# QuentinHuan/ENSEM3A_OpenCLRaytracer

Hardware: NVIDIA B200
Metric: Mrays/s (higher is better)
Workload: dtype f32

## Files before the change

ensem3a_openclraytracer_b200/_capi.py:

```python
import ctypes
import os
import subprocess

import numpy as np

_PKG = os.path.dirname(os.path.abspath(__file__))
LIB_PATH = os.path.join(_PKG, "lib", "libb200rt.so")
CSRC = os.path.join(_PKG, "csrc")

RNG_REFERENCE, RNG_PHILOX = 0, 1
TRAVERSAL_FAST, TRAVERSAL_REFERENCE, TRAVERSAL_VERIFY = 0, 1, 2
OUT_FINAL, OUT_SUMS = 0, 1
SAMPLING_REFERENCE, SAMPLING_IMPORTANCE, SAMPLING_LIGHTS = 0, 1, 2


class B200RTError(RuntimeError):
    pass


class Opts(ctypes.Structure):
    _fields_ = [("rng_mode", ctypes.c_int32), ("traversal", ctypes.c_int32), ("stack_cap", ctypes.c_int32),
                ("output", ctypes.c_int32), ("sample_begin", ctypes.c_int32), ("sample_end", ctypes.c_int32),
                ("pixel_begin", ctypes.c_int32), ("pixel_end", ctypes.c_int32), ("seed", ctypes.c_uint64),
                ("collect_stats", ctypes.c_int32), ("time_kernels", ctypes.c_int32), ("tile_row_mod", ctypes.c_int32),
# ... 26 lines not shown

DENOISE_DEFAULTS = dict(passes=5, sigma_color=0.5, sigma_normal=0.2, sigma_position=0.0)


def _denoise_params(passes=DENOISE_DEFAULTS["passes"], sigma_color=DENOISE_DEFAULTS["sigma_color"],
                    sigma_normal=DENOISE_DEFAULTS["sigma_normal"], sigma_position=DENOISE_DEFAULTS["sigma_position"]):
    return Denoise(int(passes), float(sigma_color), float(sigma_normal), float(sigma_position))


SYMBOLS = [
    "b200rt_default_opts", "b200rt_create", "b200rt_destroy", "b200rt_last_error", "b200rt_set_scene",
    "b200rt_set_materials", "b200rt_set_ibl", "b200rt_render", "b200rt_render_adaptive", "b200rt_gbuffer", "b200rt_denoise", "b200rt_render_denoised", "b200rt_render_rgb8", "b200rt_render_device", "b200rt_finalize_device",
    "b200rt_reduce_finalize_device", "b200rt_sync", "b200rt_set_stream", "b200rt_invalidate", "b200rt_primary_hits", "b200rt_trace_rays",
    "b200rt_img_processing", "b200rt_get_stats", "b200rt_math_probe", "b200rt_philox_probe", "b200rt_alloc",
    "b200rt_free", "b200rt_ipc_export",
    "b200rt_ipc_open", "b200rt_ipc_close", "b200rt_build_bvh", "b200rt_repack_probe", "b200rt_version", "b200rt_device_count",
    "b200rt_multi_create", "b200rt_multi_destroy", "b200rt_multi_last_error", "b200rt_multi_device_count",
    "b200rt_multi_context", "b200rt_multi_set_scene", "b200rt_multi_set_ibl", "b200rt_multi_invalidate",
    "b200rt_multi_render", "b200rt_multi_render_denoised", "b200rt_multi_get_stats",
]

_lib = None


def build_library(verbose=False):
    cmd = ["make", "-C", CSRC] + ([] if verbose else ["-s"])
    subprocess.check_call(cmd)
    return LIB_PATH


def load_library():
# ... 32 lines not shown
    lib.b200rt_set_stream.argtypes = [vp, vp]
    lib.b200rt_invalidate.argtypes = [vp]
    lib.b200rt_primary_hits.argtypes = [vp, vp, i32, i32, ctypes.POINTER(Opts), vp, vp]
    lib.b200rt_trace_rays.argtypes = [vp, vp, i64, ctypes.POINTER(Opts), vp, vp]
    lib.b200rt_img_processing.argtypes = [vp, vp, vp, i64, i64]
    lib.b200rt_get_stats.argtypes = [vp, ctypes.POINTER(Stats)]
    lib.b200rt_math_probe.argtypes = [vp, i32, vp, vp, i64, vp]
    lib.b200rt_philox_probe.argtypes = [vp, ctypes.POINTER(u32 * 4), u32, u32, ctypes.POINTER(u32 * 4)]
    lib.b200rt_alloc.argtypes = [vp, i64, ctypes.POINTER(vp)]
    lib.b200rt_free.argtypes = [vp, vp]
    lib.b200rt_ipc_export.argtypes = [vp, vp, vp]
    lib.b200rt_ipc_open.argtypes = [vp, vp, ctypes.POINTER(vp)]
    lib.b200rt_ipc_close.argtypes = [vp, vp]
    lib.b200rt_build_bvh.argtypes = [vp, i64, vp, i64, vp, i64, ctypes.POINTER(ctypes.c_int32)]
    lib.b200rt_repack_probe.argtypes = [vp, i64, vp, i64, vp, i64, i64, vp, i64, vp, i64, vp, vp]
    lib.b200rt_multi_create.argtypes = [ctypes.POINTER(ctypes.c_int), i32, ctypes.POINTER(vp)]
    lib.b200rt_multi_destroy.restype = None
    lib.b200rt_multi_destroy.argtypes = [vp]
    lib.b200rt_multi_last_error.restype = ctypes.c_char_p
    lib.b200rt_multi_last_error.argtypes = [vp]
    lib.b200rt_multi_device_count.argtypes = [vp]
    lib.b200rt_multi_context.restype = vp
    lib.b200rt_multi_context.argtypes = [vp, i32]
    lib.b200rt_multi_set_scene.argtypes = [vp, vp, i64, vp, i64, vp, i64, vp, i64, vp, i64, vp, i64, vp, i64]
    lib.b200rt_multi_set_ibl.argtypes = [vp, vp, i32, i32]
    lib.b200rt_multi_invalidate.argtypes = [vp]
    lib.b200rt_multi_render.argtypes = [vp, vp, vp, i32, i32, i32, i32, ctypes.POINTER(Opts), vp]
    lib.b200rt_multi_get_stats.argtypes = [vp, ctypes.POINTER(Stats)]
    for name in SYMBOLS:
        fn = getattr(lib, name)
# ... 59 lines not shown
    if rc != 0:
        raise B200RTError(f"b200rt_repack_probe failed ({rc})")
    nodes = np.zeros((int(info[0]), 8), np.uint32)
    ranks = np.zeros(face.size // 10, np.int32)
    rc = lib.b200rt_repack_probe(_ptr(vp_), vp_.size, _ptr(vn_), vn_.size, _ptr(face), face.size, int(n_materials),
                                 _ptr(bvh_), bvh_.size, _ptr(nodes), nodes.size, _ptr(ranks), _ptr(info))
    if rc != 0:
        raise B200RTError(f"b200rt_repack_probe failed ({rc})")
    d = dict(n_inner=int(info[0]), node_f4=int(info[1]), depth=int(info[2]), ref_stack_need=int(info[3]),
             canonical=bool(info[4]), fast_ok=bool(info[5]), cmax=float(info[6]), cull_abs=float(info[7]),
             grid_base=info[8:11].copy(), grid_pitch=info[11:14].copy(), root_qmin=info[14:17].copy(),
             root_qmax=info[17:20].copy(), ranks=ranks, ms_tris=float(info[20]), ms_walk=float(info[21]), ms_nodes=float(info[22]), cull_depth=int(info[23]))
    return nodes, d


class _Handle:

    _prefix = "b200rt_"

    def __del__(self):
        try:
            self.close()
        except Exception:
            pass

    def _check(self, rc, what):
        if rc != 0:
            err = getattr(self._lib, self._prefix + "last_error")(self._h).decode()
            raise B200RTError(f"{what} failed ({rc}): {err}")

# ... 257 lines not shown
```

ensem3a_openclraytracer_b200/csrc/b200rt_api.cu:

```cuda
#include <cmath>
#include <cstdarg>
#include <cstdio>
#include <cstdlib>
#include <cstring>
#include <chrono>
#include <string>
#include <type_traits>
#include <vector>

#include "../../include/b200rt.h"
#include "rt_denoise.cuh"
#include "scene_repack.h"

using namespace b200rt;

namespace {

thread_local std::string g_create_error;

struct DevBuf {
  void *p = nullptr;
  size_t cap = 0;
  bool borrowed = false;
};
// ... 66 lines not shown
  vsnprintf(buf, sizeof buf, fmt, ap);
  va_end(ap);
  if (c) c->err = buf; else g_create_error = buf;
  return code;
}

#define CU(call)                                                                                   \
  do {                                                                                             \
    cudaError_t e_ = (call);                                                                       \
    if (e_ != cudaSuccess) return fail(c, B200RT_ERR_CUDA, "%s: %s", #call, cudaGetErrorString(e_)); \
  } while (0)

}

static_assert(kRefStack == kRefStackMax, "scene_repack.h and rt_trace.cuh disagree on the exact walk's stack");
size_t b200rt::lane_smem_bytes_host(int stack_depth) { return lane_smem_bytes(stack_depth); }

namespace {

int ensure(b200rt_ctx *c, DevBuf &b, size_t bytes) {
  if (bytes == 0) bytes = 16;
  if (b.borrowed) return fail(c, B200RT_ERR_INVALID, "internal: resize of a borrowed scene buffer");
  if (b.cap >= bytes) return 0;
  if (b.p) cudaFree(b.p);
  b.p = nullptr;
  b.cap = 0;
  CU(cudaMalloc(&b.p, bytes));
  b.cap = bytes;
  return 0;
}
// ... 50 lines not shown
  F->s0 = o.sample_begin;
  F->s1 = o.sample_end;
  if (F->s1 <= 0) { F->s0 = 0; F->s1 = spp; }
  F->pixel_begin = o.pixel_begin;
  F->pixel_end = o.pixel_end;
  if (F->pixel_end <= 0) { F->pixel_begin = 0; F->pixel_end = width * height; }
  F->tile_row_mod = o.tile_row_mod;
  F->tile_row_rem = o.tile_row_rem;
  F->out_mode = o.output;
  F->rng_mode = o.rng_mode;
  F->key0 = (uint32_t)(o.seed & 0xffffffffull);
  F->key1 = (uint32_t)(o.seed >> 32);
  F->sampling = o.sampling;
}

size_t scene_smem_bytes(const b200rt_ctx *c) { return (size_t)c->scene.n_inner * 48 + (size_t)c->scene.n_tris * 48; }

bool use_smem_scene(const b200rt_ctx *c) { return c->scene.node_f4 == 3; }

int stack_entries(const b200rt_ctx *c) { return c->scene.canonical ? c->scene.cull_depth + 2 : 2; }

size_t smem_bytes(const b200rt_ctx *c, bool smem_scene) {
  return lane_smem_bytes(stack_entries(c)) + (smem_scene ? scene_smem_bytes(c) : 0);
}

int effective_stack_cap(const b200rt_ctx *c, const b200rt_opts &o);

void fill_args(b200rt_ctx *c, const FrameParams &F, const b200rt_opts &o, float *d_out, KernelArgs *A) {
  A->F = F;
  const SceneDesc &D = c->scene;
  const DevBuf *B = c->d_scene;
  SceneView &S = A->S;
  S.nodes = static_cast<const uint4 *>(B[kNodes].p);
  S.node_f4 = D.node_f4;
  S.tris = static_cast<const float4 *>(B[kTris].p);
  S.ctris = static_cast<const float4 *>(B[kCtris].p);
  S.normals = static_cast<const float4 *>(B[kNormals].p);
  S.tboxes = static_cast<const float4 *>(B[kTboxes].p);
  S.frames = static_cast<const float4 *>(B[kFrames].p);
  S.mats = static_cast<const float *>(B[kMats].p);
  S.bvh9 = static_cast<const float *>(B[kBvh9].p);
  S.leafcnt = static_cast<const int *>(B[kLeafcnt].p);
  S.root_ref = D.root_ref;
  for (int i = 0; i < 3; ++i) {
    S.grid_base[i] = D.grid_base[i];
    S.grid_pitch[i] = D.grid_pitch[i];
    S.root_w[i] = D.root_w[i];
  }
  S.cull_abs = D.cull_abs;
  S.cmax = D.cmax;
  {
    const int E = std::ilogb((1001.0f + D.cull_abs) * 1.01f) + 1;
    S.st_bias = (uint32_t)(E - 32 + 127) << 23;
    unsigned long long m = 1;
    while (m < (unsigned long long)std::max(1, D.n_inner) * (unsigned long long)std::max(1, D.node_f4)) m <<= 1;
    S.st_rmask = (uint32_t)(m - 1ull);
  }
  S.stack_cap = effective_stack_cap(c, o);
  S.fast_ok = D.fast_ok;
  A->ibl = c->ibl_tex;
  A->prim_dirk = static_cast<float4 *>(c->d_prim_dirk.p);
  A->prim_tri = static_cast<int *>(c->d_prim_tri.p);
  A->out = d_out;
  A->pA = static_cast<float4 *>(c->d_pA.p);
  A->pB = static_cast<float4 *>(c->d_pB.p);
  A->pC = static_cast<float4 *>(c->d_pC.p);
  A->pHit = static_cast<int2 *>(c->d_pHit.p);
  A->light = static_cast<const int *>(B[kLight].p);
  A->n_light = c->n_light;
  A->pS = static_cast<float4 *>(c->d_pS.p);
  A->pL = static_cast<float4 *>(c->d_pL.p);
  A->pR = static_cast<float4 *>(c->d_pR.p);
  A->list[0] = static_cast<int *>(c->d_list0.p);
  A->list[1] = static_cast<int *>(c->d_list1.p);
  A->cnt = static_cast<unsigned int *>(c->d_cnt.p);
  A->slots = static_cast<int *>(c->d_slots.p);
  A->part_count = static_cast<unsigned int *>(c->d_part_count.p);
  A->wc = nullptr;
  A->counters = c->d_counters;
  A->n_nodes = D.n_inner;
  A->n_tris = D.n_tris;
  A->stack_depth = stack_entries(c);
  A->tiles_x = (F.width + 7) / 8;
  int tiles_y = (F.height + 3) / 4;
  A->n_work = A->tiles_x * tiles_y * 32;
  A->validate = 0;
  A->ad = AdaptArgs();
}

int effective_traversal(const b200rt_ctx *c, const b200rt_opts &o) {
  if (!c->scene.canonical) return B200RT_TRAVERSAL_REFERENCE;
  return o.traversal;
}

int effective_stack_cap(const b200rt_ctx *c, const b200rt_opts &o) {
// ... 619 lines not shown

bool scene_is_cached(const b200rt_ctx *c, uint64_t h) { return c->have_scene && c->have_scene_cached && h == c->scene_hash; }

int upload_scene(b200rt_ctx *c, const Repacked &R, const SceneArgs &a, uint64_t h) {
  c->have_scene = false;
  c->have_scene_cached = false;
  c->scene_hash = 0;
  const int n_tris = R.n_tris;
  DevBuf *B = c->d_scene;
  CU(cudaSetDevice(c->device));
  if (ensure(c, B[kTris], R.tris.size() * sizeof(float4))) return B200RT_ERR_CUDA;
  if (ensure(c, B[kCtris], R.ctris.size() * sizeof(float4))) return B200RT_ERR_CUDA;
  if (ensure(c, B[kNormals], R.normals.size() * sizeof(float4))) return B200RT_ERR_CUDA;
  if (ensure(c, B[kTboxes], R.tboxes.size() * sizeof(float4))) return B200RT_ERR_CUDA;
  if (ensure(c, B[kFrames], (size_t)n_tris * kFrameVec * sizeof(float4))) return B200RT_ERR_CUDA;
  if (ensure(c, B[kNodes], R.nodes.size() * sizeof(uint4))) return B200RT_ERR_CUDA;
  if (ensure(c, B[kBvh9], (size_t)a.n_bvh * 4)) return B200RT_ERR_CUDA;
  if (ensure(c, B[kLeafcnt], R.leaf_count.size() * sizeof(int32_t))) return B200RT_ERR_CUDA;
  CU(cudaMemcpyAsync(B[kLeafcnt].p, R.leaf_count.data(), R.leaf_count.size() * sizeof(int32_t), cudaMemcpyHostToDevice, c->stream));
  CU(cudaMemcpyAsync(B[kTris].p, R.tris.data(), R.tris.size() * sizeof(float4), cudaMemcpyHostToDevice, c->stream));
  CU(cudaMemcpyAsync(B[kCtris].p, R.ctris.data(), R.ctris.size() * sizeof(float4), cudaMemcpyHostToDevice, c->stream));
  CU(cudaMemcpyAsync(B[kNormals].p, R.normals.data(), R.normals.size() * sizeof(float4), cudaMemcpyHostToDevice, c->stream));
  CU(cudaMemcpyAsync(B[kTboxes].p, R.tboxes.data(), R.tboxes.size() * sizeof(float4), cudaMemcpyHostToDevice, c->stream));
  if (!R.nodes.empty())
    CU(cudaMemcpyAsync(B[kNodes].p, R.nodes.data(), R.nodes.size() * sizeof(uint4), cudaMemcpyHostToDevice, c->stream));
  CU(cudaMemcpyAsync(B[kBvh9].p, a.bvh, (size_t)a.n_bvh * 4, cudaMemcpyHostToDevice, c->stream));
  k_tri_frames<<<(n_tris + 127) / 128, 128, 0, c->stream>>>(static_cast<const float4 *>(B[kNormals].p), n_tris,
                                                           static_cast<float4 *>(B[kFrames].p));
  CU(cudaGetLastError());
  CU(cudaStreamSynchronize(c->stream));
  c->scene = R;
  c->tri_mat = R.tri_mat;
  c->mat_hash = 0;
  c->n_mats = 0;
  int rc = b200rt_set_materials(c, a.mat, a.n_mat);
  if (rc) return rc;
  c->have_scene = true;
  c->have_scene_cached = true;
  c->scene_hash = h;
  ++c->scene_epoch;
// ... 890 lines not shown
```

ensem3a_openclraytracer_b200/csrc/rt_kernels.cuh:

```cuda
#pragma once
#include "rt_shade.cuh"
#include "rt_trace.cuh"

namespace b200rt {

constexpr int kBlock = 128;
constexpr int kShadeBlock = 128;
constexpr unsigned kChunk = 32;
constexpr int kQuorum = 12, kRefillMin = 8, kTriQuorum = 2;
constexpr int kCompactEvery = 4;
constexpr int kHitNeedsExactWalk = -2;

struct DeviceCounters {
  unsigned long long rays, box_tests, tri_tests, mismatches, samples, revalidated, exact_walks, primary_rays;
};

struct AdaptArgs {
  float2 *welford;
  int *spp_out;
  float *err_out;
  int min_spp, check_every;
  float rel_error, floor;
};

// ... 563 lines not shown
  T.Q.A = mk3(1, 1, 1); T.Q.Bn = mk3(0, 0, 0); T.Q.Bf = mk3(0, 0, 0);
  for (int a = 0; a < 3; ++a) { T.Q.sn[a] = kSelMin; T.Q.sf[a] = kSelMax; }
  int pn = 0;
  int path = -1;
  unsigned int c_next = 0, c_end = 0;
  bool exhausted = false;

  unsigned int rays = 0;
  unsigned int mism = 0;
  TraceCounters tc;
  tc.box_tests = 0; tc.tri_tests = 0;

  int thresh = kQuorum;
  for (;;) {
    for (;;) {
      const bool can = trav_active(T) && pn <= kParkCap - 2;
      if (__popc(__ballot_sync(0xffffffffu, can)) < thresh) break;
      if (can) trav_step<SMEM, STATS>(S, T, pn, parks, kBlock, st, &tc);
    }
    for (unsigned int pm = __ballot_sync(0xffffffffu, pn > 0); pm != 0u;) {
      if (pn > 0) {
        --pn;
        if (STATS) tc.tri_tests++;
        test_parked<SMEM>(S, T, parks[pn * kBlock], T.o, T.d);
      }
      pm = __ballot_sync(0xffffffffu, pn > 0);
      if (__popc(pm) < kTriQuorum) break;
    }
    const bool finished = (path >= 0) && !trav_active(T) && pn == 0;
    if (finished) {
      A.pHit[path] = make_int2(T.best.tri, __float_as_int(T.best.k));
      path = -1;
    }
    const unsigned int idle = __ballot_sync(0xffffffffu, path < 0);
    if (exhausted) {
      if (idle == 0xffffffffu) break;
      continue;
    }
    const int n_idle = __popc(idle);
    if (n_idle == 0) continue;
    if (n_idle < kRefillMin &&
        __popc(__ballot_sync(0xffffffffu, trav_active(T) && pn <= kParkCap - 2)) >= kQuorum)
      continue;
    {
      int need = n_idle;
      int rank = __popc(idle & lt_mask);
      bool want = path < 0;
      while (need > 0) {
        if (c_next == c_end) {
          unsigned int b = 0;
          if (lane == 0) b = atomicAdd(wc, kChunk);
          b = __shfl_sync(0xffffffffu, b, 0);
          if (b >= n) { exhausted = true; thresh = 1; break; }
          c_next = b;
          c_end = min(b + kChunk, n);
        }
        const int take = min(need, (int)(c_end - c_next));
// ... 146 lines not shown
```

ensem3a_openclraytracer_b200/csrc/rt_trace.cuh:

```cuda
#pragma once
#include "rt_math.cuh"

namespace b200rt {

struct SceneView {
  const uint4 *nodes;
  int node_f4;
  const float4 *tris;
  const float4 *ctris;
  const float4 *normals;
  const float4 *tboxes;
  const float4 *frames;
  const float *mats;
  const float *bvh9;
  const int *leafcnt;
  int root_ref;
  float grid_base[3];
  float grid_pitch[3];
  uint32_t root_w[3];
  float cull_abs;
  uint32_t st_bias;
  uint32_t st_rmask;
  float cmax;
  int stack_cap;
// ... 40 lines not shown
  v3 A, e1, e2;
  int mat, rank, id;
};
template <bool SMEM = false>
RT_DEV Tri load_tri(const float4 *tris, int t) {
  const float4 *p = tris + 3 * (size_t)t;
  const float4 t0 = ld4<SMEM>(p), t1 = ld4<SMEM>(p + 1), t2 = ld4<SMEM>(p + 2);
  return {mk3(t0.x, t0.y, t0.z), mk3(t0.w, t1.x, t1.y), mk3(t1.z, t1.w, t2.x), __float_as_int(t2.y), __float_as_int(t2.z),
          __float_as_int(t2.w)};
}

RT_DEV int tri_material(const SceneView &S, int tri) { return __float_as_int(__ldg(S.tris + 3 * (size_t)tri + 2).y); }
RT_DEV int tri_rank(const SceneView &S, int tri) { return __float_as_int(__ldg(S.tris + 3 * (size_t)tri + 2).z); }

template <bool SMEM>
RT_DEV void ld_node(const uint4 *p, uint4 &a, uint4 &b) {
  if (SMEM) {
    a = p[0]; b = p[1];
  } else {
    asm("ld.global.nc.v8.u32 {%0,%1,%2,%3,%4,%5,%6,%7}, [%8];"
        : "=r"(a.x), "=r"(a.y), "=r"(a.z), "=r"(a.w), "=r"(b.x), "=r"(b.y), "=r"(b.z), "=r"(b.w)
        : "l"(p));
  }
}

constexpr uint32_t kSelMax = 0x7324u;
constexpr uint32_t kSelMin = 0x7104u;
RT_DEV float plane_fq(uint32_t w, uint32_t sel) {
  uint32_t r;
  asm("prmt.b32 %0, %1, %2, %3;" : "=r"(r) : "r"(w), "r"(0x3f000000u), "r"(sel));
  return __uint_as_float(r);
}

RT_DEV float div_exact(float x, float d) {
  if (x == 0.0f && d != 0.0f && d == d) return __uint_as_float((__float_as_uint(x) ^ __float_as_uint(d)) & 0x80000000u);
  return __fdiv_rn(x, d);
}

RT_DEV bool slab_exact(v3 o, v3 d, float mnx, float mny, float mnz, float mxx, float mxy, float mxz, float *tmin,
// ... 186 lines not shown
}

struct Trav {
  v3 o, d;
  RayFast Q;
  Hit best;
  int best_rank;
  float lim;
  int cur, sp;
};

RT_DEV bool trav_active(const Trav &T) { return T.cur >= 0; }

RT_DEV float cull_limit(const SceneView &S, const Trav &T) { return __fmaf_rn(T.best.k, 1.001f, S.cull_abs); }

constexpr int kParkCap = 6;

template <bool SMEM, bool STATS>
RT_DEV void trav_begin(const SceneView &S, Trav &T, v3 o, v3 d, int &pn, uint32_t *parks, TraceCounters *cnt) {
  T.o = o; T.d = d;
  T.Q = make_rayfast(S, o, d);
  T.best.tri = -1;
  T.best.k = 1000.0f;
  T.best_rank = 0x7fffffff;
  T.lim = cull_limit(S, T);
  T.sp = 0;
  float lo, hi;
  if (STATS) cnt->box_tests++;
  slab_cons(T.Q, S.root_w[0], S.root_w[1], S.root_w[2], &lo, &hi);
  const bool go = hi >= lo;
  T.cur = go ? 0 : -1;
  if (go && S.root_ref < 0) {
    parks[0] = (uint32_t)S.root_ref;
    pn = 1;
    T.cur = -1;
  }
}

template <bool SMEM, bool STATS>
RT_DEV void trav_step(const SceneView &S, Trav &T, int &pn, uint32_t *parks, int pstride, LaneStack st,
                      TraceCounters *cnt) {
  uint4 wa, wb;
  ld_node<SMEM>(S.nodes + T.cur, wa, wb);
  const int refL = (int)wb.z, refR = (int)wb.w;
  float loL, hiL, loR, hiR;
  if (STATS) cnt->box_tests += 2;
  slab_cons(T.Q, wa.x, wa.y, wa.z, &loL, &hiL);
  slab_cons(T.Q, wa.w, wb.x, wb.y, &loR, &hiR);
  const float lim = T.lim;
  const float behind = -S.cull_abs;
  const bool goL = hiL >= loL && !(loL > lim) && !(hiL < behind);
  const bool goR = hiR >= loR && !(loR > lim) && !(hiR < behind);
  const bool leafL = goL && refL < 0, leafR = goR && refR < 0;
  const bool inL = goL && refL >= 0, inR = goR && refR >= 0;
  const bool rNear = loR < loL;
  const int refNear = rNear ? refR : refL, refFar = rNear ? refL : refR;
  const bool both = leafL && leafR;
  if (both) { parks[pn * pstride] = (uint32_t)refFar; ++pn; }
  if (leafL || leafR) { parks[pn * pstride] = (uint32_t)(both ? refNear : (leafR ? refR : refL)); ++pn; }
  if (inL && inR) {
    st.base[T.sp * st.stride] = (stack_code(S, rNear ? loL : loR) & ~S.st_rmask) | (uint32_t)refFar;
    ++T.sp;
    T.cur = refNear;
  } else if (inL || inR) {
    T.cur = inL ? refL : refR;
  } else {
    T.cur = -1;
    const uint32_t keep = stack_code(S, lim) | S.st_rmask;
    while (T.sp > 0) {
      --T.sp;
      const uint32_t e = st.base[T.sp * st.stride];
      if (e <= keep) {
        T.cur = (int)(e & S.st_rmask);
        break;
      }
    }
  }
}

template <bool SMEM>
RT_DEV void test_parked(const SceneView &S, Trav &T, uint32_t ref, v3 o, v3 d) {
  test_triangle<SMEM>(S, ~(int)ref, o, d, T.best, T.best_rank);
  T.lim = cull_limit(S, T);
}

template <bool SMEM, bool STATS>
RT_DEV Hit closest_hit_fast(const SceneView &S, v3 o, v3 d, LaneStack st, uint32_t *parks, int pstride,
                            TraceCounters *cnt) {
  if (!ray_is_fast(S, o)) return closest_hit_nodrop(S, o, d);
  Trav T;
  int pn = 0;
  trav_begin<SMEM, STATS>(S, T, o, d, pn, parks, cnt);
  while (trav_active(T) || pn > 0) {
    if (pn > 0 && (!trav_active(T) || pn > kParkCap - 2)) {
      --pn;
      if (STATS) cnt->tri_tests++;
      test_parked<SMEM>(S, T, parks[pn * pstride], o, d);
    } else {
      trav_step<SMEM, STATS>(S, T, pn, parks, pstride, st, cnt);
    }
  }
  if (T.best.tri >= 0 && !validate_winner(S, o, d, T.best.tri, T.best_rank)) return closest_hit_nodrop(S, o, d);
  return T.best;
}

template <int TRAV, bool SMEM, bool STATS>
RT_DEV Hit closest_hit(const SceneView &S, v3 o, v3 d, LaneStack st, uint32_t *parks, int pstride, TraceCounters *cnt,
                       unsigned int *mismatch) {
  if (TRAV == 0) return closest_hit_fast<SMEM, STATS>(S, o, d, st, parks, pstride, cnt);
// ... 11 lines not shown
```

ensem3a_openclraytracer_b200/csrc/scene_repack.cpp:

```cpp
#include "scene_repack.h"

#include <omp.h>

#include <algorithm>
#include <chrono>
#include <cmath>
#include <cstdio>
#include <cstdlib>
#include <cstring>

#include "../../include/b200rt.h"

namespace b200rt {

namespace {

double now_ms() {
  return std::chrono::duration<double, std::milli>(std::chrono::steady_clock::now().time_since_epoch()).count();
}

std::string fmt(const char *f, long long a = 0, long long b = 0, long long c = 0) {
  char buf[256];
  snprintf(buf, sizeof buf, f, a, b, c);
  return buf;
// ... 40 lines not shown
    if (const char *q = getenv("B200RT_HOST_THREADS")) {
      want = atoi(q);
    } else if (omp_get_max_threads() == 1) {
      const char *omp = getenv("OMP_NUM_THREADS"), *lws = getenv("LOCAL_WORLD_SIZE");
      if (omp && lws && atoi(omp) == 1 && atoi(lws) >= 1) want = std::min(16, omp_get_num_procs() / atoi(lws));
    }
    if (want >= 1) {
      saved = omp_get_max_threads();
      omp_set_num_threads(want);
    }
  }
  ~HostThreads() {
    if (saved) omp_set_num_threads(saved);
  }
};

}

int repack_scene(const float *vp, int64_t n_vp, const float *vn, int64_t n_vn, const int32_t *face, int64_t n_face,
                 int64_t n_materials, const float *bvh, int64_t n_bvh, Repacked *out, std::string *err, bool own_tree) {
  HostThreads host_threads;
  Repacked &R = *out;
  const int n_nodes = (int)(n_bvh / 9), n_tris = (int)(n_face / 10);
  const int nvp = (int)(n_vp / 3), nvn = (int)(n_vn / 3), nm = (int)n_materials;
  R.n_nodes9 = n_nodes;
  R.n_tris = n_tris;
  double t0 = now_ms();

  R.tris.resize((size_t)n_tris * 3);
  R.normals.resize((size_t)n_tris);
// ... 222 lines not shown
    return B200RT_ERR_INVALID;
  }
  R.depth = depth;
  R.cull_depth = depth;
  R.cull_tree = 0;
  R.ref_stack_need = (int)max_stack;
  if (R.ref_stack_need > kRefStackMax) canonical = false;
  double t2 = now_ms();
  R.ms_walk = t2 - t1;

  std::vector<CullNode> cull;
  if (canonical && own_tree && T(0) == -1) {
    build_cull_tree(R.tboxes.data(), n_tris, &cull, &R.cull_depth);
    R.cull_tree = 1;
  }
  if (lane_smem_bytes_host(R.cull_depth + 2) > kLaneSmemMax) canonical = false;

  Axis grid[3];
  {
    double ext[3], ext_max = 0.0;
    for (int k = 0; k < 3; ++k) {
      ext[k] = std::max(0.0, (double)bvh[5 + k] - (double)bvh[2 + k]);
      ext_max = std::max(ext_max, ext[k]);
    }
    if (ext_max == 0.0) ext_max = std::max((double)cmax, 1e-30) * 0x1p-12;
    for (int k = 0; k < 3; ++k) {
      const double e = std::max(ext[k], ext_max / 256.0);
      double widen = 0x1p-20;
      for (int attempt = 0;; ++attempt) {
        float pitch = (float)(e * (65536.0 / 32767.0) * (1.0 + 8.0 * widen));
        if (!(pitch > 0.0f) || !std::isfinite(pitch)) pitch = 1.0f;
// ... 41 lines not shown
        todo.push_back(0);
        while (!todo.empty()) {
          const int cur = todo.back();
          todo.pop_back();
          const int ch[2] = {L(cur), Rc(cur)};
          for (int k = 0; k < 2; ++k)
            if (T(ch[k]) == -1) {
              inner_id[ch[k]] = (int)order.size();
              order.push_back(ch[k]);
            }
          for (int k = 1; k >= 0; --k)
            if (T(ch[k]) == -1) todo.push_back(ch[k]);
        }
      }
      }
      std::vector<int> leaf_pos;
      if (R.cull_tree) {
        leaf_pos.assign((size_t)n_tris, -1);
        int pos = 0;
        for (size_t q = 0; q < cull.size(); ++q)
          for (int k = 0; k < 2; ++k)
            if (cull[q].ref[k] < 0) leaf_pos[(size_t)~cull[q].ref[k]] = pos++;
      }
      const int n_inner = R.cull_tree ? (int)cull.size() : (int)order.size();
      R.n_inner = n_inner;
      const int nf4 = ((size_t)n_inner * 48 + (size_t)n_tris * 48 <= kSmemSceneMax) ? 3 : 2;
      R.node_f4 = nf4;
      R.nodes.resize((size_t)n_inner * nf4);
      int outside = 0;
#pragma omp parallel for schedule(static) reduction(| : outside)
      for (int q = 0; q < n_inner; ++q) {
        const float *bl, *br;
        int32_t refl, refr;
        if (R.cull_tree) {
          const CullNode &N = cull[q];
          bl = N.box[0]; br = N.box[1];
          refl = N.ref[0] < 0 ? ~leaf_pos[(size_t)~N.ref[0]] : N.ref[0] * nf4;
          refr = N.ref[1] < 0 ? ~leaf_pos[(size_t)~N.ref[1]] : N.ref[1] * nf4;
        } else {
          const int cur = order[q];
          const int l = L(cur), r = Rc(cur);
          bl = bvh + 9 * (size_t)l + 2; br = bvh + 9 * (size_t)r + 2;
          refl = T(l) != -1 ? ~T(l) : (int32_t)(inner_id[l] * nf4);
          refr = T(r) != -1 ? ~T(r) : (int32_t)(inner_id[r] * nf4);
        }
        uint32_t wl[3], wr[3];
        for (int k = 0; k < 3; ++k)
          if (!quantise(grid[k], bl[k], bl[3 + k], &wl[k]) || !quantise(grid[k], br[k], br[3 + k], &wr[k])) outside |= 1;
        Repacked::u4 a, b;
        a.x = wl[0]; a.y = wl[1]; a.z = wl[2]; a.w = wr[0];
        b.x = wr[1]; b.y = wr[2];
        b.z = (uint32_t)refl;
        b.w = (uint32_t)refr;
        R.nodes[(size_t)nf4 * q + 0] = a;
        R.nodes[(size_t)nf4 * q + 1] = b;
        if (nf4 == 3) R.nodes[(size_t)nf4 * q + 2] = Repacked::u4{0, 0, 0, 0};
      }
      if (R.cull_tree) {
        R.ctris.resize((size_t)n_tris * 3);
#pragma omp parallel for schedule(static)
        for (int t = 0; t < n_tris; ++t) {
          const size_t p = (size_t)leaf_pos[(size_t)t];
          R.ctris[3 * p] = R.tris[3 * (size_t)t];
          R.ctris[3 * p + 1] = R.tris[3 * (size_t)t + 1];
          Repacked::f4 t2 = R.tris[3 * (size_t)t + 2];
          t2.w = as_float((uint32_t)t);
          R.ctris[3 * p + 2] = t2;
        }
      }
      if (outside) {
        R.canonical = false;
        R.nodes.clear();
        R.n_inner = 0;
        R.node_f4 = 2;
      }
    }
  }
  if (R.ctris.size() != R.tris.size() || !R.cull_tree || !R.canonical) {
    R.ctris.resize(R.tris.size());
#pragma omp parallel for schedule(static)
    for (int t = 0; t < n_tris; ++t) {
      R.ctris[3 * (size_t)t] = R.tris[3 * (size_t)t];
      R.ctris[3 * (size_t)t + 1] = R.tris[3 * (size_t)t + 1];
      Repacked::f4 t2 = R.tris[3 * (size_t)t + 2];
      t2.w = as_float((uint32_t)t);
      R.ctris[3 * (size_t)t + 2] = t2;
    }
  }
  R.ms_nodes = now_ms() - t2;
  return 0;
}

}
// ... 12 lines not shown
  info[0] = (float)R.n_inner; info[1] = (float)R.node_f4; info[2] = (float)R.depth; info[3] = (float)R.ref_stack_need;
  info[4] = R.canonical ? 1.0f : 0.0f; info[5] = (float)R.fast_ok; info[6] = R.cmax; info[7] = R.cull_abs;
  for (int k = 0; k < 3; ++k) {
    info[8 + k] = R.grid_base[k]; info[11 + k] = R.grid_pitch[k];
    info[14 + k] = (float)(R.root_w[k] & 0xffffu); info[17 + k] = (float)(R.root_w[k] >> 16);
  }
  info[20] = (float)R.ms_tris; info[21] = (float)R.ms_walk; info[22] = (float)R.ms_nodes; info[23] = (float)R.cull_depth;
  if (rank_out)
    for (int t = 0; t < R.n_tris; ++t) memcpy(&rank_out[t], &R.tris[3 * (size_t)t + 2].z, 4);
  if (nodes_out) {
    if (n_nodes_out < (int64_t)R.n_inner * 8) return B200RT_ERR_INVALID;
    for (int q = 0; q < R.n_inner; ++q) {
      const b200rt::Repacked::u4 &a = R.nodes[(size_t)R.node_f4 * q], &b = R.nodes[(size_t)R.node_f4 * q + 1];
      uint32_t *o = nodes_out + 8 * (size_t)q;
      o[0] = a.x; o[1] = a.y; o[2] = a.z; o[3] = a.w; o[4] = b.x; o[5] = b.y; o[6] = b.z; o[7] = b.w;
      for (int k = 6; k < 8; ++k)
        if ((int32_t)o[k] < 0) {
          uint32_t id;
          memcpy(&id, &R.ctris[3 * (size_t)~(int32_t)o[k] + 2].w, 4);
          o[k] = (uint32_t)~(int32_t)id;
        }
    }
  }
  return 0;
}
```

ensem3a_openclraytracer_b200/csrc/scene_repack.h:

```cpp
#pragma once
#include <cstdint>
#include <memory>
#include <string>
#include <vector>

namespace b200rt {

template <class T>
struct raw_alloc : std::allocator<T> {
  template <class U> struct rebind { using other = raw_alloc<U>; };
  raw_alloc() = default;
  template <class U> raw_alloc(const raw_alloc<U> &) {}
  template <class U> void construct(U *p) noexcept { ::new (static_cast<void *>(p)) U; }
  template <class U, class... A> void construct(U *p, A &&...a) { ::new (static_cast<void *>(p)) U(std::forward<A>(a)...); }
};
template <class T> using raw_vector = std::vector<T, raw_alloc<T>>;

struct SceneDesc {
  int n_nodes9 = 0, n_inner = 0, n_tris = 0;
  int node_f4 = 2;
  int depth = 0, ref_stack_need = 0;
  int cull_depth = 0;
  bool canonical = true;
  int root_ref = 0;
  float grid_base[3] = {0, 0, 0}, grid_pitch[3] = {1, 1, 1};
  uint32_t root_w[3] = {0x7fff0000u, 0x7fff0000u, 0x7fff0000u};
  float cull_abs = 0.0f, cmax = 0.0f;
  int fast_ok = 0;
  float root_box[6] = {0, 0, 0, 0, 0, 0};
};

struct Repacked : SceneDesc {
  struct f4 { float x, y, z, w; };
  struct u4 { uint32_t x, y, z, w; };
  raw_vector<u4> nodes;
  raw_vector<f4> tris, normals, tboxes;
  raw_vector<f4> ctris;
  std::vector<int32_t> tri_mat;
  raw_vector<int32_t> leaf_count;
  int cull_tree = 0;
  double ms_tris = 0, ms_walk = 0, ms_nodes = 0;
};

constexpr size_t kSmemSceneMax = 48 * 1024;
constexpr int kRefStackMax = 64;
constexpr size_t kLaneSmemMax = 96 * 1024;

struct CullNode {
  float box[2][6];
  int32_t ref[2];
};

void build_cull_tree(const Repacked::f4 *tboxes, int n_tris, std::vector<CullNode> *out, int *depth_out);

size_t lane_smem_bytes_host(int stack_depth);

int repack_scene(const float *vp, int64_t n_vp, const float *vn, int64_t n_vn, const int32_t *face, int64_t n_face,
                 int64_t n_materials, const float *bvh, int64_t n_bvh, Repacked *out, std::string *err, bool own_tree = true);

}
```

include/b200rt.h:

```cpp
#ifndef B200RT_H
#define B200RT_H

#include <stdint.h>

#ifdef __cplusplus
extern "C" {
#endif

typedef struct b200rt_ctx b200rt_ctx;

typedef enum {
  B200RT_OK = 0,
  B200RT_ERR_INVALID = -1,
  B200RT_ERR_CUDA = -2,
  B200RT_ERR_NO_SCENE = -3,
  B200RT_ERR_UNSUPPORTED = -4
} b200rt_status;

#define B200RT_RNG_REFERENCE 0
#define B200RT_RNG_PHILOX 1

#define B200RT_TRAVERSAL_FAST 0
#define B200RT_TRAVERSAL_REFERENCE 1
#define B200RT_TRAVERSAL_VERIFY 2
// ... 150 lines not shown
                           int64_t n_face_data, const float *material_data, int64_t n_material_data,
                           const int32_t *light_data, int64_t n_light_data, const float *bvh, int64_t n_bvh);
int b200rt_multi_set_ibl(b200rt_multi *m, const uint8_t *rgba, int width, int height);
int b200rt_multi_invalidate(b200rt_multi *m);
int b200rt_multi_render(b200rt_multi *m, const float *cam, const float *env, int width, int height, int spp,
                        int max_bounce, const b200rt_opts *opts, float *out_rgb);
int b200rt_multi_render_denoised(b200rt_multi *m, const float *cam, const float *env, int width, int height, int spp,
                                 int max_bounce, const b200rt_opts *opts, const b200rt_denoise_params *dn, float *out_rgb,
                                 float *out_noisy);
int b200rt_multi_get_stats(const b200rt_multi *m, b200rt_stats *stats);

int b200rt_repack_probe(const float *vertex_p, int64_t n_vertex_p, const float *vertex_n, int64_t n_vertex_n,
                        const int32_t *face_data, int64_t n_face_data, int64_t n_materials, const float *bvh,
                        int64_t n_bvh, uint32_t *nodes_out, int64_t n_nodes_out, int32_t *rank_out, float *info_out);

const char *b200rt_version(void);

int b200rt_device_count(void);

#ifdef __cplusplus
}
#endif
#endif
```

Measured before the change: 5434.

## Collapse binary cull BVH into 4-wide nodes with sorted child traversal

Converts the binary quantized BVH into a 4-wide BVH by repeatedly opening the largest-area inner child, and lays out the new nodes in 4 or 5 uint4 words with an empty-slot sentinel. The traversal step now tests four child boxes per node, sorts them by entry distance with a small sorting network, parks leaf hits and pushes the farther inner children onto the stack. The park buffer and the park thresholds grow to absorb up to four leaves per step. The aim is fewer node fetches and a shallower traversal, at the cost of more box tests per step, more registers, and a larger per-lane shared-memory footprint.

Result: no change. 5469 (median of 6 runs) (+0.7%).

```diff
diff --git a/ensem3a_openclraytracer_b200/_capi.py b/ensem3a_openclraytracer_b200/_capi.py
--- a/ensem3a_openclraytracer_b200/_capi.py
+++ b/ensem3a_openclraytracer_b200/_capi.py
@@ -64,7 +64,7 @@
     "b200rt_reduce_finalize_device", "b200rt_sync", "b200rt_set_stream", "b200rt_invalidate", "b200rt_primary_hits", "b200rt_trace_rays",
     "b200rt_img_processing", "b200rt_get_stats", "b200rt_math_probe", "b200rt_philox_probe", "b200rt_alloc",
     "b200rt_free", "b200rt_ipc_export",
-    "b200rt_ipc_open", "b200rt_ipc_close", "b200rt_build_bvh", "b200rt_repack_probe", "b200rt_version", "b200rt_device_count",
+    "b200rt_ipc_open", "b200rt_ipc_close", "b200rt_build_bvh", "b200rt_repack_probe", "b200rt_repack_probe_wide", "b200rt_version", "b200rt_device_count",
     "b200rt_multi_create", "b200rt_multi_destroy", "b200rt_multi_last_error", "b200rt_multi_device_count",
     "b200rt_multi_context", "b200rt_multi_set_scene", "b200rt_multi_set_ibl", "b200rt_multi_invalidate",
     "b200rt_multi_render", "b200rt_multi_render_denoised", "b200rt_multi_get_stats",
@@ -127,6 +127,7 @@
     lib.b200rt_ipc_close.argtypes = [vp, vp]
     lib.b200rt_build_bvh.argtypes = [vp, i64, vp, i64, vp, i64, ctypes.POINTER(ctypes.c_int32)]
     lib.b200rt_repack_probe.argtypes = [vp, i64, vp, i64, vp, i64, i64, vp, i64, vp, i64, vp, vp]
+    lib.b200rt_repack_probe_wide.argtypes = [vp, i64, vp, i64, vp, i64, i64, vp, i64, vp, i64, vp]
     lib.b200rt_multi_create.argtypes = [ctypes.POINTER(ctypes.c_int), i32, ctypes.POINTER(vp)]
     lib.b200rt_multi_destroy.restype = None
     lib.b200rt_multi_destroy.argtypes = [vp]
@@ -216,6 +217,21 @@
     return nodes, d
 
 
+def repack_probe_wide(vertex_p, vertex_n, face_data, n_materials, bvh):
+    lib = load_library()
+    vp_, vn_, face, bvh_ = _f32(vertex_p), _f32(vertex_n), _i32(face_data), _f32(bvh)
+    info = np.zeros(3, np.int32)
+    args = (_ptr(vp_), vp_.size, _ptr(vn_), vn_.size, _ptr(face), face.size, int(n_materials), _ptr(bvh_), bvh_.size)
+    rc = lib.b200rt_repack_probe_wide(*args, None, 0, _ptr(info))
+    if rc != 0:
+        raise B200RTError(f"b200rt_repack_probe_wide failed ({rc})")
+    nodes = np.zeros((int(info[0]), 16), np.uint32)
+    rc = lib.b200rt_repack_probe_wide(*args, _ptr(nodes), nodes.size, _ptr(info))
+    if rc != 0:
+        raise B200RTError(f"b200rt_repack_probe_wide failed ({rc})")
+    return nodes, dict(n_wide=int(info[0]), wide_f4=int(info[1]), stack_bound=int(info[2]))
+
+
 class _Handle:
 
     _prefix = "b200rt_"
diff --git a/ensem3a_openclraytracer_b200/csrc/b200rt_api.cu b/ensem3a_openclraytracer_b200/csrc/b200rt_api.cu
--- a/ensem3a_openclraytracer_b200/csrc/b200rt_api.cu
+++ b/ensem3a_openclraytracer_b200/csrc/b200rt_api.cu
@@ -104,6 +104,7 @@
 }
 
 static_assert(kRefStack == kRefStackMax, "scene_repack.h and rt_trace.cuh disagree on the exact walk's stack");
+static_assert(kEmptyRef == (int)kWideEmpty, "scene_repack.h and rt_trace.cuh disagree on the unused-slot ref");
 size_t b200rt::lane_smem_bytes_host(int stack_depth) { return lane_smem_bytes(stack_depth); }
 
 namespace {
@@ -184,11 +185,13 @@
   F->sampling = o.sampling;
 }
 
-size_t scene_smem_bytes(const b200rt_ctx *c) { return (size_t)c->scene.n_inner * 48 + (size_t)c->scene.n_tris * 48; }
-
-bool use_smem_scene(const b200rt_ctx *c) { return c->scene.node_f4 == 3; }
-
-int stack_entries(const b200rt_ctx *c) { return c->scene.canonical ? c->scene.cull_depth + 2 : 2; }
+size_t scene_smem_bytes(const b200rt_ctx *c) {
+  return (size_t)c->scene.n_wide * 16 * c->scene.wide_f4 + (size_t)c->scene.n_tris * 48;
+}
+
+bool use_smem_scene(const b200rt_ctx *c) { return c->scene.wide_f4 == 5; }
+
+int stack_entries(const b200rt_ctx *c) { return c->scene.canonical ? c->scene.wide_stack + 2 : 2; }
 
 size_t smem_bytes(const b200rt_ctx *c, bool smem_scene) {
   return lane_smem_bytes(stack_entries(c)) + (smem_scene ? scene_smem_bytes(c) : 0);
@@ -202,7 +205,7 @@
   const DevBuf *B = c->d_scene;
   SceneView &S = A->S;
   S.nodes = static_cast<const uint4 *>(B[kNodes].p);
-  S.node_f4 = D.node_f4;
+  S.node_f4 = D.wide_f4;
   S.tris = static_cast<const float4 *>(B[kTris].p);
   S.ctris = static_cast<const float4 *>(B[kCtris].p);
   S.normals = static_cast<const float4 *>(B[kNormals].p);
@@ -223,7 +226,7 @@
     const int E = std::ilogb((1001.0f + D.cull_abs) * 1.01f) + 1;
     S.st_bias = (uint32_t)(E - 32 + 127) << 23;
     unsigned long long m = 1;
-    while (m < (unsigned long long)std::max(1, D.n_inner) * (unsigned long long)std::max(1, D.node_f4)) m <<= 1;
+    while (m < (unsigned long long)std::max(1, D.n_wide) * (unsigned long long)D.wide_f4) m <<= 1;
     S.st_rmask = (uint32_t)(m - 1ull);
   }
   S.stack_cap = effective_stack_cap(c, o);
@@ -248,7 +251,7 @@
   A->part_count = static_cast<unsigned int *>(c->d_part_count.p);
   A->wc = nullptr;
   A->counters = c->d_counters;
-  A->n_nodes = D.n_inner;
+  A->n_nodes = D.n_wide;
   A->n_tris = D.n_tris;
   A->stack_depth = stack_entries(c);
   A->tiles_x = (F.width + 7) / 8;
@@ -898,7 +901,7 @@
   if (ensure(c, B[kNormals], R.normals.size() * sizeof(float4))) return B200RT_ERR_CUDA;
   if (ensure(c, B[kTboxes], R.tboxes.size() * sizeof(float4))) return B200RT_ERR_CUDA;
   if (ensure(c, B[kFrames], (size_t)n_tris * kFrameVec * sizeof(float4))) return B200RT_ERR_CUDA;
-  if (ensure(c, B[kNodes], R.nodes.size() * sizeof(uint4))) return B200RT_ERR_CUDA;
+  if (ensure(c, B[kNodes], R.wnodes.size() * sizeof(uint4))) return B200RT_ERR_CUDA;
   if (ensure(c, B[kBvh9], (size_t)a.n_bvh * 4)) return B200RT_ERR_CUDA;
   if (ensure(c, B[kLeafcnt], R.leaf_count.size() * sizeof(int32_t))) return B200RT_ERR_CUDA;
   CU(cudaMemcpyAsync(B[kLeafcnt].p, R.leaf_count.data(), R.leaf_count.size() * sizeof(int32_t), cudaMemcpyHostToDevice, c->stream));
@@ -906,8 +909,8 @@
   CU(cudaMemcpyAsync(B[kCtris].p, R.ctris.data(), R.ctris.size() * sizeof(float4), cudaMemcpyHostToDevice, c->stream));
   CU(cudaMemcpyAsync(B[kNormals].p, R.normals.data(), R.normals.size() * sizeof(float4), cudaMemcpyHostToDevice, c->stream));
   CU(cudaMemcpyAsync(B[kTboxes].p, R.tboxes.data(), R.tboxes.size() * sizeof(float4), cudaMemcpyHostToDevice, c->stream));
-  if (!R.nodes.empty())
-    CU(cudaMemcpyAsync(B[kNodes].p, R.nodes.data(), R.nodes.size() * sizeof(uint4), cudaMemcpyHostToDevice, c->stream));
+  if (!R.wnodes.empty())
+    CU(cudaMemcpyAsync(B[kNodes].p, R.wnodes.data(), R.wnodes.size() * sizeof(uint4), cudaMemcpyHostToDevice, c->stream));
   CU(cudaMemcpyAsync(B[kBvh9].p, a.bvh, (size_t)a.n_bvh * 4, cudaMemcpyHostToDevice, c->stream));
   k_tri_frames<<<(n_tris + 127) / 128, 128, 0, c->stream>>>(static_cast<const float4 *>(B[kNormals].p), n_tris,
                                                            static_cast<float4 *>(B[kFrames].p));
diff --git a/ensem3a_openclraytracer_b200/csrc/rt_kernels.cuh b/ensem3a_openclraytracer_b200/csrc/rt_kernels.cuh
--- a/ensem3a_openclraytracer_b200/csrc/rt_kernels.cuh
+++ b/ensem3a_openclraytracer_b200/csrc/rt_kernels.cuh
@@ -601,7 +601,7 @@
   int thresh = kQuorum;
   for (;;) {
     for (;;) {
-      const bool can = trav_active(T) && pn <= kParkCap - 2;
+      const bool can = trav_active(T) && pn <= kParkCap - 4;
       if (__popc(__ballot_sync(0xffffffffu, can)) < thresh) break;
       if (can) trav_step<SMEM, STATS>(S, T, pn, parks, kBlock, st, &tc);
     }
@@ -627,7 +627,7 @@
     const int n_idle = __popc(idle);
     if (n_idle == 0) continue;
     if (n_idle < kRefillMin &&
-        __popc(__ballot_sync(0xffffffffu, trav_active(T) && pn <= kParkCap - 2)) >= kQuorum)
+        __popc(__ballot_sync(0xffffffffu, trav_active(T) && pn <= kParkCap - 4)) >= kQuorum)
       continue;
     {
       int need = n_idle;
diff --git a/ensem3a_openclraytracer_b200/csrc/rt_trace.cuh b/ensem3a_openclraytracer_b200/csrc/rt_trace.cuh
--- a/ensem3a_openclraytracer_b200/csrc/rt_trace.cuh
+++ b/ensem3a_openclraytracer_b200/csrc/rt_trace.cuh
@@ -78,7 +78,7 @@
 RT_DEV int tri_rank(const SceneView &S, int tri) { return __float_as_int(__ldg(S.tris + 3 * (size_t)tri + 2).z); }
 
 template <bool SMEM>
-RT_DEV void ld_node(const uint4 *p, uint4 &a, uint4 &b) {
+RT_DEV void ld_half(const uint4 *p, uint4 &a, uint4 &b) {
   if (SMEM) {
     a = p[0]; b = p[1];
   } else {
@@ -87,6 +87,8 @@
         : "l"(p));
   }
 }
+
+constexpr int kEmptyRef = (int)0x80000000u;
 
 constexpr uint32_t kSelMax = 0x7324u;
 constexpr uint32_t kSelMin = 0x7104u;
@@ -303,7 +305,7 @@
 
 RT_DEV float cull_limit(const SceneView &S, const Trav &T) { return __fmaf_rn(T.best.k, 1.001f, S.cull_abs); }
 
-constexpr int kParkCap = 6;
+constexpr int kParkCap = 8;
 
 template <bool SMEM, bool STATS>
 RT_DEV void trav_begin(const SceneView &S, Trav &T, v3 o, v3 d, int &pn, uint32_t *parks, TraceCounters *cnt) {
@@ -326,36 +328,70 @@
   }
 }
 
+RT_DEV float slot_key(const SceneView &S, const Trav &T, uint32_t wx, uint32_t wy, uint32_t wz) {
+  float lo, hi;
+  slab_cons(T.Q, wx, wy, wz, &lo, &hi);
+  const bool go = hi >= lo && !(lo > T.lim) && !(hi < -S.cull_abs);
+  return go ? lo : INFINITY;
+}
+
+RT_DEV void sort2(float &ki, int &ri, float &kj, int &rj) {
+  const bool sw = kj < ki;
+  const float k = sw ? kj : ki;
+  const int r = sw ? rj : ri;
+  kj = sw ? ki : kj;
+  rj = sw ? ri : rj;
+  ki = k;
+  ri = r;
+}
+
 template <bool SMEM, bool STATS>
 RT_DEV void trav_step(const SceneView &S, Trav &T, int &pn, uint32_t *parks, int pstride, LaneStack st,
                       TraceCounters *cnt) {
-  uint4 wa, wb;
-  ld_node<SMEM>(S.nodes + T.cur, wa, wb);
-  const int refL = (int)wb.z, refR = (int)wb.w;
-  float loL, hiL, loR, hiR;
-  if (STATS) cnt->box_tests += 2;
-  slab_cons(T.Q, wa.x, wa.y, wa.z, &loL, &hiL);
-  slab_cons(T.Q, wa.w, wb.x, wb.y, &loR, &hiR);
-  const float lim = T.lim;
-  const float behind = -S.cull_abs;
-  const bool goL = hiL >= loL && !(loL > lim) && !(hiL < behind);
-  const bool goR = hiR >= loR && !(loR > lim) && !(hiR < behind);
-  const bool leafL = goL && refL < 0, leafR = goR && refR < 0;
-  const bool inL = goL && refL >= 0, inR = goR && refR >= 0;
-  const bool rNear = loR < loL;
-  const int refNear = rNear ? refR : refL, refFar = rNear ? refL : refR;
-  const bool both = leafL && leafR;
-  if (both) { parks[pn * pstride] = (uint32_t)refFar; ++pn; }
-  if (leafL || leafR) { parks[pn * pstride] = (uint32_t)(both ? refNear : (leafR ? refR : refL)); ++pn; }
-  if (inL && inR) {
-    st.base[T.sp * st.stride] = (stack_code(S, rNear ? loL : loR) & ~S.st_rmask) | (uint32_t)refFar;
-    ++T.sp;
-    T.cur = refNear;
-  } else if (inL || inR) {
-    T.cur = inL ? refL : refR;
-  } else {
-    T.cur = -1;
-    const uint32_t keep = stack_code(S, lim) | S.st_rmask;
+  uint4 wa, wb, wc, wd;
+  ld_half<SMEM>(S.nodes + T.cur, wa, wb);
+  ld_half<SMEM>(S.nodes + T.cur + 2, wc, wd);
+  float k0 = slot_key(S, T, wa.x, wa.y, wa.z), k1 = slot_key(S, T, wa.w, wb.x, wb.y);
+  int r0 = (int)wb.z, r1 = (int)wb.w;
+  int r2 = (int)wd.z, r3 = (int)wd.w;
+  float k2 = slot_key(S, T, wc.x, wc.y, wc.z), k3 = slot_key(S, T, wc.w, wd.x, wd.y);
+  k2 = r2 == kEmptyRef ? INFINITY : k2;
+  k3 = r3 == kEmptyRef ? INFINITY : k3;
+  if (STATS) cnt->box_tests += 2 + (r2 != kEmptyRef) + (r3 != kEmptyRef);
+  sort2(k0, r0, k1, r1);
+  sort2(k2, r2, k3, r3);
+  sort2(k0, r0, k2, r2);
+  sort2(k1, r1, k3, r3);
+  sort2(k1, r1, k2, r2);
+  const float ks[4] = {k0, k1, k2, k3};
+  const int rs[4] = {r0, r1, r2, r3};
+  bool go[4], inner[4];
+#pragma unroll
+  for (int i = 0; i < 4; ++i) {
+    go[i] = ks[i] != INFINITY;
+    inner[i] = go[i] && rs[i] >= 0;
+  }
+#pragma unroll
+  for (int i = 3; i >= 0; --i)
+    if (go[i] && !inner[i]) {
+      parks[pn * pstride] = (uint32_t)rs[i];
+      ++pn;
+    }
+  const bool nearer[4] = {false, inner[0], inner[0] || inner[1], inner[0] || inner[1] || inner[2]};
+#pragma unroll
+  for (int i = 3; i >= 1; --i) {
+    const uint32_t e = (stack_code(S, ks[i]) & ~S.st_rmask) | (uint32_t)rs[i];
+    if (inner[i] && nearer[i]) {
+      st.base[T.sp * st.stride] = e;
+      ++T.sp;
+    }
+  }
+  int next = -1;
+#pragma unroll
+  for (int i = 3; i >= 0; --i) next = inner[i] ? rs[i] : next;
+  T.cur = next;
+  if (next < 0) {
+    const uint32_t keep = stack_code(S, T.lim) | S.st_rmask;
     while (T.sp > 0) {
       --T.sp;
       const uint32_t e = st.base[T.sp * st.stride];
@@ -381,7 +417,7 @@
   int pn = 0;
   trav_begin<SMEM, STATS>(S, T, o, d, pn, parks, cnt);
   while (trav_active(T) || pn > 0) {
-    if (pn > 0 && (!trav_active(T) || pn > kParkCap - 2)) {
+    if (pn > 0 && (!trav_active(T) || pn > kParkCap - 4)) {
       --pn;
       if (STATS) cnt->tri_tests++;
       test_parked<SMEM>(S, T, parks[pn * pstride], o, d);
diff --git a/ensem3a_openclraytracer_b200/csrc/scene_repack.cpp b/ensem3a_openclraytracer_b200/csrc/scene_repack.cpp
--- a/ensem3a_openclraytracer_b200/csrc/scene_repack.cpp
+++ b/ensem3a_openclraytracer_b200/csrc/scene_repack.cpp
@@ -78,6 +78,109 @@
     if (saved) omp_set_num_threads(saved);
   }
 };
+
+void collapse_wide(Repacked &R) {
+  const int nf4 = R.node_f4, n_tris = R.n_tris;
+  struct Kid {
+    const uint32_t *w;
+    int32_t ref;
+  };
+  auto kid_of = [&](int q, int s) {
+    const uint32_t *r = reinterpret_cast<const uint32_t *>(&R.nodes[(size_t)nf4 * q]);
+    return Kid{r + 3 * s, (int32_t)r[6 + s]};
+  };
+  auto area = [&](const uint32_t *w) {
+    double e[3];
+    for (int k = 0; k < 3; ++k) e[k] = (double)((w[k] >> 16) - (w[k] & 0xffffu)) * (double)R.grid_pitch[k];
+    return e[0] * e[1] + e[1] * e[2] + e[2] * e[0];
+  };
+  struct Wide {
+    uint32_t w[4][3];
+    int32_t ref[4];
+  };
+  std::vector<Wide> wide(1);
+  std::vector<int> start(1, 0), above(1, 0);
+  std::vector<int> todo(1, 0);
+  int bound = 0;
+  while (!todo.empty()) {
+    const int wi = todo.back();
+    todo.pop_back();
+    Kid kid[4] = {kid_of(start[wi], 0), kid_of(start[wi], 1)};
+    int n = 2;
+    while (n < 4) {
+      int open = -1;
+      double best = -1.0;
+      for (int i = 0; i < n; ++i)
+        if (kid[i].ref >= 0 && area(kid[i].w) >= best) {
+          best = area(kid[i].w);
+          open = i;
+        }
+      if (open < 0) break;
+      const int q = kid[open].ref / nf4;
+      for (int i = n; i > open + 1; --i) kid[i] = kid[i - 1];
+      kid[open] = kid_of(q, 0);
+      kid[open + 1] = kid_of(q, 1);
+      ++n;
+    }
+    Wide W;
+    const int first = (int)wide.size(), up = above[wi];
+    int inner = 0;
+    for (int i = 0; i < 4; ++i) {
+      for (int k = 0; k < 3; ++k) W.w[i][k] = i < n ? kid[i].w[k] : 0u;
+      const int32_t r = i < n ? kid[i].ref : (int32_t)kWideEmpty;
+      W.ref[i] = r;
+      if (i < n && r >= 0) {
+        W.ref[i] = first + inner++;
+        start.push_back(r / nf4);
+      }
+    }
+    wide[wi] = W;
+    const int here = up + std::max(0, inner - 1);
+    bound = std::max(bound, here);
+    wide.resize((size_t)first + inner);
+    above.resize((size_t)first + inner, here);
+    for (int j = first + inner - 1; j >= first; --j) todo.push_back(j);
+  }
+  const int n_wide = (int)wide.size();
+  std::vector<int> leaf_pos((size_t)n_tris, -1);
+  int pos = 0;
+  for (const Wide &W : wide)
+    for (int i = 0; i < 4; ++i)
+      if (W.ref[i] < 0 && (uint32_t)W.ref[i] != kWideEmpty) leaf_pos[(size_t)~W.ref[i]] = pos++;
+  for (int t = 0; t < n_tris; ++t)
+    if (leaf_pos[(size_t)t] < 0) leaf_pos[(size_t)t] = pos++;
+  const int wf4 = ((size_t)n_wide * 80 + (size_t)n_tris * 48 <= kSmemSceneMax) ? 5 : 4;
+  R.n_wide = n_wide;
+  R.wide_f4 = wf4;
+  R.wide_stack = bound;
+  R.wnodes.resize((size_t)n_wide * wf4);
+#pragma omp parallel for schedule(static)
+  for (int q = 0; q < n_wide; ++q) {
+    const Wide &W = wide[q];
+    uint32_t ref[4];
+    for (int i = 0; i < 4; ++i) {
+      const int32_t r = W.ref[i];
+      ref[i] = (uint32_t)r == kWideEmpty ? kWideEmpty : (uint32_t)(r >= 0 ? r * wf4 : ~leaf_pos[(size_t)~r]);
+    }
+    Repacked::u4 *o = &R.wnodes[(size_t)wf4 * q];
+    for (int h = 0; h < 2; ++h) {
+      const uint32_t *a = W.w[2 * h], *b = W.w[2 * h + 1];
+      o[2 * h] = Repacked::u4{a[0], a[1], a[2], b[0]};
+      o[2 * h + 1] = Repacked::u4{b[1], b[2], ref[2 * h], ref[2 * h + 1]};
+    }
+    if (wf4 == 5) o[4] = Repacked::u4{0, 0, 0, 0};
+  }
+  R.ctris.resize((size_t)n_tris * 3);
+#pragma omp parallel for schedule(static)
+  for (int t = 0; t < n_tris; ++t) {
+    const size_t p = (size_t)leaf_pos[(size_t)t];
+    R.ctris[3 * p] = R.tris[3 * (size_t)t];
+    R.ctris[3 * p + 1] = R.tris[3 * (size_t)t + 1];
+    Repacked::f4 t2 = R.tris[3 * (size_t)t + 2];
+    t2.w = as_float((uint32_t)t);
+    R.ctris[3 * p + 2] = t2;
+  }
+}
 
 }
 
@@ -330,7 +433,6 @@
     build_cull_tree(R.tboxes.data(), n_tris, &cull, &R.cull_depth);
     R.cull_tree = 1;
   }
-  if (lane_smem_bytes_host(R.cull_depth + 2) > kLaneSmemMax) canonical = false;
 
   Axis grid[3];
   {
@@ -402,14 +504,6 @@
         }
       }
       }
-      std::vector<int> leaf_pos;
-      if (R.cull_tree) {
-        leaf_pos.assign((size_t)n_tris, -1);
-        int pos = 0;
-        for (size_t q = 0; q < cull.size(); ++q)
-          for (int k = 0; k < 2; ++k)
-            if (cull[q].ref[k] < 0) leaf_pos[(size_t)~cull[q].ref[k]] = pos++;
-      }
       const int n_inner = R.cull_tree ? (int)cull.size() : (int)order.size();
       R.n_inner = n_inner;
       const int nf4 = ((size_t)n_inner * 48 + (size_t)n_tris * 48 <= kSmemSceneMax) ? 3 : 2;
@@ -423,8 +517,8 @@
         if (R.cull_tree) {
           const CullNode &N = cull[q];
           bl = N.box[0]; br = N.box[1];
-          refl = N.ref[0] < 0 ? ~leaf_pos[(size_t)~N.ref[0]] : N.ref[0] * nf4;
-          refr = N.ref[1] < 0 ? ~leaf_pos[(size_t)~N.ref[1]] : N.ref[1] * nf4;
+          refl = N.ref[0] < 0 ? N.ref[0] : N.ref[0] * nf4;
+          refr = N.ref[1] < 0 ? N.ref[1] : N.ref[1] * nf4;
         } else {
           const int cur = order[q];
           const int l = L(cur), r = Rc(cur);
@@ -444,27 +538,20 @@
         R.nodes[(size_t)nf4 * q + 1] = b;
         if (nf4 == 3) R.nodes[(size_t)nf4 * q + 2] = Repacked::u4{0, 0, 0, 0};
       }
-      if (R.cull_tree) {
-        R.ctris.resize((size_t)n_tris * 3);
-#pragma omp parallel for schedule(static)
-        for (int t = 0; t < n_tris; ++t) {
-          const size_t p = (size_t)leaf_pos[(size_t)t];
-          R.ctris[3 * p] = R.tris[3 * (size_t)t];
-          R.ctris[3 * p + 1] = R.tris[3 * (size_t)t + 1];
-          Repacked::f4 t2 = R.tris[3 * (size_t)t + 2];
-          t2.w = as_float((uint32_t)t);
-          R.ctris[3 * p + 2] = t2;
-        }
-      }
-      if (outside) {
+      if (!outside) collapse_wide(R);
+      if (outside || lane_smem_bytes_host(R.wide_stack + 2) > kLaneSmemMax) {
         R.canonical = false;
         R.nodes.clear();
         R.n_inner = 0;
         R.node_f4 = 2;
-      }
-    }
-  }
-  if (R.ctris.size() != R.tris.size() || !R.cull_tree || !R.canonical) {
+        R.wnodes.clear();
+        R.n_wide = 0;
+        R.wide_f4 = 4;
+        R.wide_stack = 0;
+      }
+    }
+  }
+  if (R.n_wide == 0) {
     R.ctris.resize(R.tris.size());
 #pragma omp parallel for schedule(static)
     for (int t = 0; t < n_tris; ++t) {
@@ -507,12 +594,39 @@
       const b200rt::Repacked::u4 &a = R.nodes[(size_t)R.node_f4 * q], &b = R.nodes[(size_t)R.node_f4 * q + 1];
       uint32_t *o = nodes_out + 8 * (size_t)q;
       o[0] = a.x; o[1] = a.y; o[2] = a.z; o[3] = a.w; o[4] = b.x; o[5] = b.y; o[6] = b.z; o[7] = b.w;
-      for (int k = 6; k < 8; ++k)
-        if ((int32_t)o[k] < 0) {
+    }
+  }
+  return 0;
+}
+
+extern "C" int b200rt_repack_probe_wide(const float *vp, int64_t n_vp, const float *vn, int64_t n_vn, const int32_t *face,
+                                        int64_t n_face, int64_t n_materials, const float *bvh, int64_t n_bvh,
+                                        uint32_t *nodes_out, int64_t n_nodes_out, int32_t *info) {
+  if (!vp || !vn || !face || !bvh || !info || n_vp <= 0 || n_vp % 3 || n_vn <= 0 || n_vn % 3 || n_face <= 0 || n_face % 10 ||
+      n_bvh <= 0 || n_bvh % 9 || n_materials <= 0)
+    return B200RT_ERR_INVALID;
+  b200rt::Repacked R;
+  std::string msg;
+  const char *own = getenv("B200RT_CULL_TREE");
+  int rc = b200rt::repack_scene(vp, n_vp, vn, n_vn, face, n_face, n_materials, bvh, n_bvh, &R, &msg, !(own && own[0] == '0'));
+  if (rc) return rc;
+  info[0] = R.n_wide; info[1] = R.wide_f4; info[2] = R.wide_stack;
+  if (nodes_out) {
+    if (n_nodes_out < (int64_t)R.n_wide * 16) return B200RT_ERR_INVALID;
+    for (int q = 0; q < R.n_wide; ++q) {
+      uint32_t *o = nodes_out + 16 * (size_t)q;
+      memcpy(o, &R.wnodes[(size_t)R.wide_f4 * q], 64);
+      for (int k : {6, 7, 14, 15}) {
+        const int32_t r = (int32_t)o[k];
+        if ((uint32_t)r == b200rt::kWideEmpty) continue;
+        if (r >= 0) {
+          o[k] = (uint32_t)(r / R.wide_f4);
+        } else {
           uint32_t id;
-          memcpy(&id, &R.ctris[3 * (size_t)~(int32_t)o[k] + 2].w, 4);
+          memcpy(&id, &R.ctris[3 * (size_t)~r + 2].w, 4);
           o[k] = (uint32_t)~(int32_t)id;
         }
+      }
     }
   }
   return 0;
diff --git a/ensem3a_openclraytracer_b200/csrc/scene_repack.h b/ensem3a_openclraytracer_b200/csrc/scene_repack.h
--- a/ensem3a_openclraytracer_b200/csrc/scene_repack.h
+++ b/ensem3a_openclraytracer_b200/csrc/scene_repack.h
@@ -21,6 +21,9 @@
   int node_f4 = 2;
   int depth = 0, ref_stack_need = 0;
   int cull_depth = 0;
+  int n_wide = 0;
+  int wide_f4 = 4;
+  int wide_stack = 0;
   bool canonical = true;
   int root_ref = 0;
   float grid_base[3] = {0, 0, 0}, grid_pitch[3] = {1, 1, 1};
@@ -34,6 +37,7 @@
   struct f4 { float x, y, z, w; };
   struct u4 { uint32_t x, y, z, w; };
   raw_vector<u4> nodes;
+  raw_vector<u4> wnodes;
   raw_vector<f4> tris, normals, tboxes;
   raw_vector<f4> ctris;
   std::vector<int32_t> tri_mat;
@@ -45,6 +49,7 @@
 constexpr size_t kSmemSceneMax = 48 * 1024;
 constexpr int kRefStackMax = 64;
 constexpr size_t kLaneSmemMax = 96 * 1024;
+constexpr uint32_t kWideEmpty = 0x80000000u;
 
 struct CullNode {
   float box[2][6];
diff --git a/include/b200rt.h b/include/b200rt.h
--- a/include/b200rt.h
+++ b/include/b200rt.h
@@ -188,6 +188,10 @@
                         const int32_t *face_data, int64_t n_face_data, int64_t n_materials, const float *bvh,
                         int64_t n_bvh, uint32_t *nodes_out, int64_t n_nodes_out, int32_t *rank_out, float *info_out);
 
+int b200rt_repack_probe_wide(const float *vertex_p, int64_t n_vertex_p, const float *vertex_n, int64_t n_vertex_n,
+                             const int32_t *face_data, int64_t n_face_data, int64_t n_materials, const float *bvh,
+                             int64_t n_bvh, uint32_t *nodes_out, int64_t n_nodes_out, int32_t *info_out);
+
 const char *b200rt_version(void);
 
 int b200rt_device_count(void);
```
